# HaoZhongkai/DPOT

Hardware: AMD Instinct MI355X
Metric: PDE samples/sec (128^2 x10 -> 1 rollout step), DPOT-Tiny train step (higher is better)
Workload: dtype f32

## Files before the change

dpot_amd/_lib.py:

```python
from __future__ import annotations

import ctypes as C
import os
import threading

HERE = os.path.dirname(os.path.abspath(__file__))
LIB_PATH = os.environ.get("DPOT_HIP_LIB") or os.path.join(HERE, "lib", "libdpot_hip.so")

c_fp = C.c_void_p
c_i = C.c_int
c_i64 = C.c_int64
c_f = C.c_float
c_d = C.c_double


class GemmDesc(C.Structure):
    _fields_ = [
        ("A", c_fp), ("B", c_fp), ("C", c_fp),
        ("M", C.c_int32), ("N", C.c_int32), ("K", C.c_int32),
        ("batch", C.c_int32),
        ("transA", C.c_int32), ("transB", C.c_int32),
        ("lda", C.c_int32), ("ldb", C.c_int32), ("ldc", C.c_int32),
        ("strideA", c_i64), ("strideB", c_i64), ("strideC", c_i64),
        ("bias", c_fp), ("strideBias", c_i64),
# ... 76 lines not shown
    "dpot_groupnorm_ws_elems": (c_i64, [c_i] * 4),
    "dpot_groupnorm_fwd": (c_i, [c_fp] * 7 + [c_i] * 4 + [c_f, c_fp]),
    "dpot_groupnorm_bwd": (c_i, [c_fp] * 11 + [c_i] * 4 + [c_fp]),
    "dpot_groupnorm_bwd_packs_supported": (c_i, [c_i] * 3),
    "dpot_groupnorm_bwd_packs_rows": (c_i, [c_i] * 4),
    "dpot_groupnorm_bwd_packs": (c_i, [c_fp] * 12 + [c_i] * 4 + [c_fp]),
    "dpot_groupnorm_param_grads": (c_i, [C.c_void_p] * 3 + [c_i] * 3 + [c_fp]),
    "dpot_afno_fused_supported": (c_i, [c_i] * 7),
    "dpot_afno_fused_fwd": (c_i, [c_fp] * 19 + [c_i] * 9 + [c_f, c_fp]),
    "dpot_gn_dft_supported": (c_i, [c_i] * 4),
    "dpot_gn_rfft2": (c_i, [c_fp] * 6 + [c_i] * 8 + [c_f, c_fp]),
    "dpot_irfft2_gn": (c_i, [c_fp] * 12 + [c_i] * 9 + [c_f, c_fp]),
    "dpot_gn_bwd_rfft2": (c_i, [c_fp] * 8 + [c_i] * 9 + [c_fp]),
    "dpot_irfft2_gn_bwd": (c_i, [c_fp] * 9 + [c_i] * 9 + [c_fp]),
    "dpot_patchify": (c_i, [c_fp] * 5 + [c_i] * 6 + [c_fp]),
    "dpot_unpatchify": (c_i, [c_fp] * 2 + [c_i] * 6 + [c_fp]),
    "dpot_pixel_shuffle": (c_i, [c_fp] * 2 + [c_i] * 6 + [c_fp]),
    "dpot_copy2d_pad": (c_i, [c_fp, c_i, c_i, c_fp, c_i, c_i, c_fp]),
    "dpot_transpose2d": (c_i, [c_fp, c_fp, c_i, c_i, c_i, c_fp]),
    "dpot_colsum_parts": (c_i, [c_i]),
    "dpot_colsum": (c_i, [c_fp, c_i, c_i, c_i, c_fp, c_fp, c_fp]),
    "dpot_colsum_scatter": (c_i, [c_fp, c_i, c_i, c_i, c_fp, c_i, C.POINTER(C.c_int), C.POINTER(C.c_int),
                                  C.POINTER(C.c_void_p), c_fp]),
    "dpot_group_rowsum": (c_i, [c_fp, c_fp] + [c_i] * 4 + [c_fp]),
    "dpot_small_linear_supported": (c_i, [c_i] * 3),
    "dpot_small_linear": (c_i, [c_fp, c_i, c_fp, c_i, c_fp, c_fp, c_fp] + [c_i] * 5 + [c_fp]),
    "dpot_token_mean": (c_i, [c_fp, c_fp] + [c_i] * 3 + [c_fp]),
    "dpot_token_mean_bwd": (c_i, [c_fp] * 3 + [c_i] * 3 + [c_fp]),
    "dpot_bias_add": (c_i, [c_fp] * 3 + [c_i, c_i, c_fp]),
    "dpot_scale_shift": (c_i, [c_fp] * 4 + [c_i] * 3 + [c_fp]),
    "dpot_scale_shift_bwd": (c_i, [c_fp] * 6 + [c_i] * 3 + [c_fp]),
    "dpot_timeagg_scale_w": (c_i, [c_fp] * 4 + [c_i, c_i, c_fp]),
    "dpot_timeagg_scale_w_bwd": (c_i, [c_fp] * 6 + [c_i, c_i, c_fp]),
    "dpot_out_tail_partial_rows": (c_i, [c_i] * 4),
    "dpot_out_tail_partial_cols": (c_i, []),
    "dpot_out_tail_fwd": (c_i, [c_fp] * 6 + [c_i] * 6 + [c_fp]),
    "dpot_out_tail_bwd": (c_i, [c_fp] * 7 + [c_i] * 6 + [c_fp]),
    "dpot_rel_l2_chunks": (c_i, [c_i, c_i]),
    "dpot_rel_l2_fwd": (c_i, [c_fp] * 5 + [c_i] * 4 + [c_fp]),
    "dpot_rel_l2_bwd": (c_i, [c_fp] * 6 + [c_i] * 4 + [c_fp]),
    "dpot_sumsq": (c_i, [c_fp, c_i64, c_fp, c_fp, c_i, c_fp]),
    "dpot_adam_step": (c_i, [c_fp] * 4 + [c_i64, c_fp, c_fp, c_f, c_fp]),
    "dpot_adam_stage": (c_i, [c_fp, c_fp, c_f, c_d, c_d, c_f, c_f, c_f, c_i, c_fp]),
    "dpot_lamb_chunk_elems": (c_i, []),
    "dpot_lamb_step": (c_i, [c_fp] * 5 + [c_fp, c_f, c_fp, c_i, c_fp, c_i, c_fp, c_fp, c_i, c_fp]),
    "dpot_lamb_stage": (c_i, [c_fp, c_fp, c_d, c_d, c_d, c_f, c_f, c_f, c_f, c_i, c_i, c_fp]),
    "dpot_cls_ce_fwd": (c_i, [c_fp] * 4 + [c_i, c_i, c_fp]),
    "dpot_cls_ce_bwd": (c_i, [c_fp] * 5 + [c_i, c_i, c_fp]),
    "dpot_rel_l2_combine": (c_i, [c_fp, c_fp, c_i64, c_i, c_i, c_i, c_fp, c_fp]),
    "dpot_metrics_accum": (c_i, [c_fp] * 4 + [c_i, c_fp, c_f, c_i64, c_i64, c_i64, c_fp]),
    "dpot_noise_chunks": (c_i, [c_i, c_i]),
    "dpot_noise_inject": (c_i, [c_fp] * 4 + [c_f] + [c_i] * 3 + [c_fp]),
    "dpot_noise_inject_rng": (c_i, [c_fp] * 4 + [c_f] + [c_i] * 3 + [c_fp]),
    "dpot_noise_inject_bwd": (c_i, [c_fp] * 7 + [c_f] + [c_i] * 3 + [c_fp]),
    "dpot_window_slide": (c_i, [c_fp] * 3 + [c_i64] + [c_i] * 3 + [c_fp]),
    "dpot_window_slide_bwd": (c_i, [c_fp] * 3 + [c_i64] + [c_i] * 3 + [c_fp]),
    "dpot_resize_pad_window": (c_i, [c_fp, c_i, c_fp, c_fp] + [c_i] * 6 + [c_fp]),
    "dpot_spectral_resize_pad": (c_i, [c_i, c_i]),
    "dpot_spectral_resize": (c_i, [c_fp] * 7 + [c_i] * 6 + [c_fp]),
    "dpot_eval_metrics_pad": (c_i, [c_i, c_i]),
    "dpot_eval_metrics_max_size": (c_i, [c_i]),
    "dpot_eval_metrics_acc_elems": (c_i64, [c_i] * 4),
    "dpot_eval_metrics_stats": (c_i, [c_fp] * 9 + [c_i] * 4 + [c_fp]),
    "dpot_eval_metrics_finalize": (c_i, [c_fp] * 3 + [c_i] * 5 + [c_fp]),
    "dpot_panel_pack_weights": (c_i, [c_fp, c_i, c_i, c_fp]),
    "dpot_layout_jobs": (c_i, [c_fp, c_i, c_i64, c_fp]),
# ... 71 lines not shown
```

dpot_amd/build.py:

```python
from __future__ import annotations

import os
import shutil
import subprocess
import sys
from concurrent.futures import ThreadPoolExecutor

HERE = os.path.dirname(os.path.abspath(__file__))
CSRC = os.path.join(HERE, "csrc")
LIBDIR = os.path.join(HERE, "lib")
LIB = os.path.join(LIBDIR, "libdpot_hip.so")
SOURCES = ["core.hip", "gemm.hip", "gemm_panel.hip", "gemm_tn.hip", "gemm_bf16p.hip", "afno_mlp.hip", "afno_mlp6.hip", "afno_fused.hip", "dft.hip", "norm.hip", "gn_dft.hip", "misc.hip", "loss_opt.hip", "metrics.hip", "tail.hip", "data.hip", "embed.hip", "resize.hip", "evalmetrics.hip"]
FLAGS = ["--offload-arch=gfx950", "-O3", "-std=c++17", "-fPIC", "-Wall", "-Wno-unused-function",
         "-Wno-pass-failed"]
EXTRA_FLAGS = {"afno_mlp6.hip": ["-fno-slp-vectorize"]}


def _hipcc() -> str:
    for cand in (os.environ.get("HIPCC"), shutil.which("hipcc"), "/opt/rocm/bin/hipcc"):
        if cand and os.path.exists(cand):
            return cand
    raise RuntimeError("hipcc not found (need ROCm >= 7.0 to build the gfx950 kernels)")


def _stale(target: str, deps) -> bool:
    if not os.path.exists(target):
        return True
    t = os.path.getmtime(target)
    return any(os.path.getmtime(d) > t for d in deps)


def build(force: bool = False, verbose: bool = True) -> str:
    hipcc = _hipcc()
    os.makedirs(LIBDIR, exist_ok=True)
    hdrs = [os.path.join(CSRC, "common.h"), os.path.join(CSRC, "dft_fast.h"), os.path.join(CSRC, "gemm_split.h"), os.path.join(CSRC, "gemm_epi.h"), os.path.join(CSRC, "gemm_bf16p_common.h"), os.path.join(os.path.dirname(HERE), "include", "dpot_hip.h")]
    objs, jobs = [], []
    for src in SOURCES:
        s = os.path.join(CSRC, src)
        o = os.path.join(LIBDIR, src.replace(".hip", ".o"))
        objs.append(o)
        if force or _stale(o, [s] + hdrs):
            jobs.append([hipcc] + FLAGS + EXTRA_FLAGS.get(src, []) + ["-c", s, "-o", o])

    def run(cmd):
        if verbose:
# ... 17 lines not shown
```

dpot_amd/functional.py:

```python
from __future__ import annotations

import os
from collections import OrderedDict
from typing import Optional

import torch

from . import ops
from .ops import EPI_ACT, EPI_DACT

Tensor = torch.Tensor


def _pad4(n: int) -> int:
    return (n + 3) // 4 * 4


class _Sink:
    __slots__ = ("fp", "i")

    def __init__(self, param: Optional[Tensor], needed: bool):
        s = getattr(param, "_dpot_grad_slot", None) if (needed and param is not None) else None
        self.fp, self.i = s if s is not None else (None, -1)
        if self.fp is not None:
# ... 44 lines not shown
    return [_Sink(p, ctx.needs_input_grad[first_index + k]) for k, p in enumerate(params)]


def embed_grid_matrix(gx, gy, gt, X: int, Y: int, T: int, Cc: int, P: int):
    z = torch.zeros(1, X, Y, T, Cc, dtype=torch.float32, device=gx.device)
    return ops.patchify(z, gx, gy, gt, P)[:, Cc * P * P:].contiguous()


def embed_layout_jobs(pos, w0, b0, w2, b2):
    hid, E = w0.shape[0], w2.shape[0]
    K0 = w0[0].numel()
    hidp = _pad4(hid)
    tok = pos.shape[2] * pos.shape[3]
    return [(w0, None, (1, hidp, K0), (1, hid, K0), (0, K0, 1)),
            (b0, None, (1, 1, hidp), (1, 1, hid), (0, 0, 1)),
            (w2, None, (1, E, hidp), (1, E, hid), (0, hid, 1)),
            (pos, b2, (1, tok, E), (1, tok, E), (0, 1, tok))]


def embed_derived(pos, w0, b0, w2, b2, taw, tagamma, tt, T: int, grid=None, layouts=None):
    hid, E = w0.shape[0], w2.shape[0]
    K0 = w0[0].numel()
    hidp = _pad4(hid)
    tok = pos.shape[2] * pos.shape[3]
    dev = pos.device
    if layouts is not None:
        w0p, b0p, w2p, posb = layouts[0].view(hidp, K0), layouts[1].view(hidp), layouts[2].view(E, hidp), layouts[3].view(tok, E)
    else:
        w0p = ops.copy2d_pad(w0, hid, K0, hidp, K0)
        b0p = ops.copy2d_pad(b0, 1, hid, 1, hidp).view(hidp)
        w2p = ops.copy2d_pad(w2, E, hid, E, hidp)
        posT = ops.transpose2d(pos, 1, E, tok).view(tok, E)
        posb = ops.bias_add(posT, b2)
    ws = ops.timeagg_scale_w(taw, tagamma, tt) if tagamma is not None else taw
    V = torch.empty(T * hidp, E, dtype=torch.float32, device=dev)
    ops.gemm(w2p, ws, V, hidp, E, E, transA=True, lda=hidp, ldb=E, ldc=E, batch=T, strideA=0, strideB=E * E,
             strideC=hidp * E)
    wsum = ops.colsum(ws, T, E * E).view(E, E)
    cc = torch.empty(tok, E, dtype=torch.float32, device=dev)
    ops.gemm(posb, wsum, cc, tok, E, E, lda=E, ldb=E, ldc=E)
    wfrag = bt = None
    if grid is not None:
        kg = grid.shape[1]
        wfrag = ops.embed_pack_w0(w0)
        bt = torch.empty(grid.shape[0], hidp, dtype=torch.float32, device=dev)
        ops.gemm(grid, w0p[:, K0 - kg:], bt, grid.shape[0], hidp, kg, transB=True, lda=kg, ldb=K0, ldc=hidp, bias=b0p)
    return w0p, b0p, w2p, posb, ws, V, wsum, cc, wfrag, bt, grid


class EmbedFn(torch.autograd.Function):

    @staticmethod
    def forward(ctx, x, pos, w0, b0, w2, b2, taw, tagamma, gx, gy, gt, tt, P: int, act: int, derived=None):
        ops.capture_precision(ctx)
        x = x.contiguous()
        B, X, Y, T, Cc = x.shape
        h, w = X // P, Y // P
        tok = h * w
        hid, E = w0.shape[0], w2.shape[0]
        K0 = (Cc + 3) * P * P
        hidp = _pad4(hid)
        dev = x.device
        M = B * tok

        implicit = derived is not None and derived[8] is not None
        A0 = None if implicit else ops.patchify(x, gx, gy, gt, P)
        if derived is None:
            derived = embed_derived(pos, w0, b0, w2, b2, taw, tagamma, tt, T)
        w0p, b0p, w2p, posb, ws, V, wsum, cc, wfrag, bt, grid = derived
        if implicit:
            Hh, Hpre = ops.embed_fwd(x, wfrag, bt, hidp, act)
        else:
            Hh, Hpre = ops.linear_fwd(A0, w0p, b0p, act=act, save_pre=True)
        Yl = torch.empty(M, E, dtype=torch.float32, device=dev)
        ops.gemm(Hh, V, Yl, M, E, T * hidp, lda=T * hidp, ldb=E, ldc=E, res=cc, ldres=E, res_mod=tok)
        ctx.implicit = implicit
        ctx.save_for_backward(x if implicit else A0, Hpre, Hh, w0p, w2p, ws, V, wsum, posb, taw, tagamma, tt,
                              grid if implicit else x.new_empty(0))
        ctx.dims = (B, X, Y, T, Cc, P, h, w, hid, hidp, E, K0, act)
        ctx.sinks = _sinks(ctx, (pos, w0, b0, w2, b2, taw, tagamma), 1)
        ctx.weights_epoch = _epoch_of(ctx.sinks)
        return Yl.view(B, tok, E)

    @staticmethod
    @ops.with_ctx_precision
    def backward(ctx, dY):
        _check_epoch(ctx, "EmbedFn")
        A0, Hpre, Hh, w0p, w2p, ws, V, wsum, posb, taw, tagamma, tt, grid = ctx.saved_tensors
        B, X, Y, T, Cc, P, h, w, hid, hidp, E, K0, act = ctx.dims
        s_pos, s_w0, s_b0, s_w2, s_b2, s_taw, s_gamma = ctx.sinks
        tok = h * w
        M, M0 = B * tok, B * tok * T
        dev = dY.device
        dY = dY.contiguous().view(M, E)
        dHpre = torch.empty(M0, hidp, dtype=torch.float32, device=dev)
        ops.gemm(dY, V, dHpre, M, T * hidp, E, transB=True, lda=E, ldb=E, ldc=T * hidp, act=act, mode=EPI_DACT,
                 aux=Hpre, ldaux=T * hidp)
        dV = torch.empty(T * hidp, E, dtype=torch.float32, device=dev)
        ops.gemm(Hh, dY, dV, T * hidp, E, M, transA=True, lda=T * hidp, ldb=E, ldc=E,
                 splitk=ops.auto_splitk(T * hidp, E, M, tn=True))
        dc = ops.group_rowsum(dY, B, tok, 1, E)
        dwsum = torch.empty(E, E, dtype=torch.float32, device=dev)
        ops.gemm(posb, dc, dwsum, E, E, tok, transA=True, lda=E, ldb=E, ldc=E, splitk=ops.auto_splitk(E, E, tok, tn=True))
        dposb = torch.empty(tok, E, dtype=torch.float32, device=dev)
        ops.gemm(dc, wsum, dposb, tok, E, E, transB=True, lda=E, ldb=E, ldc=E)
        dpos = s_pos.done(ops.transpose2d(dposb, 1, tok, E, out=s_pos.out()).view(1, E, h, w))
        db2 = s_b2.done(ops.colsum(dposb, tok, E, out=s_b2.out()))
        dw2_t = torch.empty(T, E, hidp, dtype=torch.float32, device=dev)
        ops.gemm(ws, dV, dw2_t, E, hidp, E, transB=True, lda=E, ldb=E, ldc=hidp, batch=T, strideA=E * E,
                 strideB=hidp * E, strideC=E * hidp)
        dw2p = ops.colsum(dw2_t, T, E * hidp).view(E, hidp)
        dw2 = s_w2.done(ops.copy2d_pad(dw2p, E, hidp, E, hid, out=s_w2.out()).view(E, hid, 1, 1))
        dws = s_taw.out() if tagamma is None else None
        dws = ops._out(dws, (T, E, E), dev)
        ops.gemm(w2p, dV, dws, E, E, hidp, lda=hidp, ldb=E, ldc=E, batch=T, strideA=0, strideB=hidp * E,
                 strideC=E * E, res=dwsum, ldres=E, strideRes=0)
        if tagamma is not None:
            dtaw, dgamma = ops.timeagg_scale_w_bwd(dws, taw, tagamma, tt, out_dw=s_taw.out(),
                                                   out_dgamma=s_gamma.out())
            dtaw, dgamma = s_taw.done(dtaw), s_gamma.done(dgamma)
        else:
            dtaw, dgamma = s_taw.done(dws), None
        if ctx.implicit:
            db0 = s_b0.done(ops.colsum(dHpre, M0, hid, ld=hidp, out=s_b0.out()))
            dw0 = ops._out(s_w0.out(), (hid, K0), dev)
            ops.embed_wgrad(A0, dHpre, dw0, hid)
            dHs = ops.group_rowsum(dHpre, B, tok * T, 1, hidp)
            kg = grid.shape[1]
            ops.gemm(dHs, grid, dw0[:, K0 - kg:], hid, kg, tok * T, transA=True, lda=hidp, ldb=kg, ldc=K0)
            dw0 = s_w0.done(dw0.view(hid, Cc + 3, P, P))
        elif hid == hidp:
            dw0p, db0 = ops.linear_bwd_wb(dHpre, A0, None, s_b0.out())
            db0 = s_b0.done(db0)
        else:
            db0 = s_b0.done(ops.colsum(dHpre, M0, hid, ld=hidp, out=s_b0.out()))
            dw0p = ops.linear_bwd_weight(dHpre, A0)
        if not ctx.implicit:
            dw0 = s_w0.done(ops.copy2d_pad(dw0p, hidp, K0, hid, K0, out=s_w0.out()).view(hid, Cc + 3, P, P))
        dx = None
        if ctx.needs_input_grad[0]:
            dA0 = ops.linear_bwd_data(dHpre, w0p)
            dx = ops.unpatchify(dA0, B, X, Y, T, Cc, P)
        return dx, dpos, dw0, db0, dw2, db2, dtaw, dgamma, None, None, None, None, None, None, None


X6_MIN_FLOP = 3.0e9


def mlp_pack_kind(E: int, mh: int, M: Optional[int] = None) -> Optional[str]:
    eff = ops.effective_mlp_precision()
    Mq = 128 if M is None else M
    bf_ok = ops.gemm_bf16p_supported(Mq, mh, E) and ops.gemm_bf16p_supported(Mq, E, mh)
    if bf_ok and eff == ops.GEMM_BF16:
        return "bf16"
    if eff == ops.GEMM_F32 and ops.panel_enabled() and ops.gemm_panel_supported(Mq, mh, E) \
            and ops.gemm_panel_supported(Mq, E, mh):
        return "f32"
    return None


# ... 635 lines not shown
```

dpot_amd/ops.py:

```python
from __future__ import annotations

import ctypes as C
import contextlib
import functools
import threading
import os
from typing import Optional, Tuple

import torch

from . import _lib
from ._lib import GemmDesc, check

Tensor = torch.Tensor

ACT_IDS = {None: 0, "none": 0, "gelu": 1, "tanh": 2, "sigmoid": 3, "relu": 4, "leaky_relu": 5, "softplus": 6,
           "ELU": 7, "silu": 8}
EPI_LINEAR, EPI_ACT, EPI_DACT, EPI_AFNO_WGRAD = 0, 1, 2, 3
GEMM_F32, GEMM_BF16X6, GEMM_AUTO, GEMM_BF16 = 0, 1, 2, 3
_PRECISIONS = {"f32": GEMM_F32, "bf16x6": GEMM_BF16X6, "auto": GEMM_AUTO, "bf16": GEMM_BF16}
_gemm_precision = _PRECISIONS[os.environ.get("DPOT_GEMM_PRECISION", "f32")]


def set_gemm_precision(name: str) -> None:
# ... 72 lines not shown
        with precision_scope(getattr(ctx, "gemm_precision", None), getattr(ctx, "mlp_precision", None)):
            return backward(ctx, *grads)
    return wrapper


def capture_precision(ctx) -> None:
    ctx.gemm_precision = _cur_gemm()
    ctx.mlp_precision = effective_mlp_precision()


def effective_mlp_precision() -> int:
    m = _cur_mlp()
    return m if m is not None else _cur_gemm()


def mlp_precision() -> Optional[int]:
    return _cur_mlp()


TUNE_KEYS = {
    "mixer": (3, "AFNO mixer MLP: 3 = three-product fused kernel (afno_mlp3), 4 = four-product fused kernel (afno_mlp2), "
                 "0 = two generic GEMM launches"),
    "afno_layer": (-1, "one-launch AFNO layer forward (afno_fused_fwd): -1 = where it measured faster (>= 80 % full last "
                       "round of (sample, block) workgroups), 0 = never, 1 = wherever supported"),
    "gn_fuse": (1, "0 = GroupNorm as its own kernels: not fused with the mixer's DFTs, never applied on the load of its consumer"),
    "panel": (1, "0 = generic GEMM kernels instead of the pre-packed-weight panel GEMM, the token-contraction weight-gradient "
                 "kernels (gemm_tn) and their two-layer launches"),
    "wgrad_gauss": (1, "0 = four-product AFNO weight gradients instead of the three-product forms"),
    "bf16p_bd": (1, "0 = the LDS-DMA bf16 GEMM kernels of rounds 2-3 for every launch instead of the B-direct kernels"),
    "bf16p_shape": (1, "0 = none of the bf16 GEMM shape heuristics: 128 x 256 tiles only, column-major tile order, eight waves, "
                       "un-paired weight gradients"),
    "packs": (1, "0 = bf16 packs by separate pack passes only: none from the one-launch AFNO layer, the GroupNorm backward or Adam"),
    "pack_both": (1, "0 = bf16 channel MLP without the pack-both path (one pack pass per operand form, fp32 pre-activation saved)"),
    "fused_small": (1, "0 = separate small launches: per-block reduce launches, eight layout launches, torch ops for the cls head"),
    "embed_implicit": (1, "0 = explicit patch matrix + GEMM instead of the implicit-GEMM patch embedding"),
    "mixer6": (1, "bf16x6 mixer kernel afno_mlp6 under gemm_precision 'auto' / 'bf16x6': 1 = where it measured faster (96 channels "
                  "per block: DPOT-L), 2 = wherever supported (also 128), 0 = never (the fp32 matrix-core kernels)"),
}


_tune_parsed = ("", {})


def _parse_tune():
    global _tune_parsed
    env = os.environ.get("DPOT_TUNE", "")
    if env == _tune_parsed[0]:
        return _tune_parsed[1]
    out = {}
    for kv in env.split(","):
        kv = kv.strip()
        if not kv:
            continue
        k, _, v = kv.partition("=")
        if k not in TUNE_KEYS:
            raise ValueError(f"DPOT_TUNE: unknown key {k!r} (known: {', '.join(TUNE_KEYS)})")
        out[k] = int(v)
    _tune_parsed = (env, out)
    return out


def tune(key: str, default: Optional[int] = None) -> int:
    d = TUNE_KEYS[key][0] if default is None else default
    return _parse_tune().get(key, d)


def _stream() -> int:
# ... 837 lines not shown


def tile_vec(v: Tensor, reps: int) -> Tensor:
    N = v.numel()
    y = torch.empty(reps * N, dtype=torch.float32, device=v.device)
    check(_lib.load().dpot_bias_add(None, v.data_ptr(), y.data_ptr(), reps, N, _stream()), "tile_vec")
    return y


def scale_shift(x: Tensor, scale: Tensor, shift: Tensor) -> Tensor:
    B, T, E = x.shape
    y = torch.empty_like(x)
    check(_lib.load().dpot_scale_shift(x.data_ptr(), scale.data_ptr(), shift.data_ptr(), y.data_ptr(), B, T, E,
                                       _stream()), "scale_shift")
    return y


def scale_shift_bwd(dy: Tensor, x: Tensor, scale: Tensor):
    B, T, E = x.shape
    dx = torch.empty_like(x)
    dscale = torch.empty(B, E, dtype=torch.float32, device=x.device)
    dshift = torch.empty_like(dscale)
    check(_lib.load().dpot_scale_shift_bwd(dy.data_ptr(), x.data_ptr(), scale.data_ptr(), dx.data_ptr(),
                                           dscale.data_ptr(), dshift.data_ptr(), B, T, E, _stream()), "scale_shift_bwd")
    return dx, dscale, dshift


def timeagg_scale_w(w: Tensor, gamma: Tensor, tt: Tensor) -> Tensor:
    T, E, _ = w.shape
    ws = torch.empty_like(w)
    check(_lib.load().dpot_timeagg_scale_w(w.data_ptr(), gamma.data_ptr(), tt.data_ptr(), ws.data_ptr(), T, E,
                                           _stream()), "timeagg_scale_w")
    return ws


def timeagg_scale_w_bwd(dws: Tensor, w: Tensor, gamma: Tensor, tt: Tensor, out_dw: Optional[Tensor] = None,
                        out_dgamma: Optional[Tensor] = None) -> Tuple[Tensor, Tensor]:
    T, E, _ = w.shape
    dw = _out(out_dw, (T, E, E), w.device)
    dgamma = _out(out_dgamma, (1, E), w.device)
    check(_lib.load().dpot_timeagg_scale_w_bwd(dws.data_ptr(), w.data_ptr(), gamma.data_ptr(), tt.data_ptr(),
                                               dw.data_ptr(), dgamma.data_ptr(), T, E, _stream()),
          "timeagg_scale_w_bwd")
    return dw, dgamma


def out_tail_supported(old: int, co: int, n_pixels: int) -> bool:
    return old == 32 and 0 < co <= 32 and n_pixels % 32 == 0


def out_tail_pad(w4: Tensor, b4: Tensor, co: int) -> Tuple[Tensor, Tensor]:
    return copy2d_pad(w4, co, 32, 32, 32), copy2d_pad(b4, 1, co, 1, 32).view(32)


def out_tail_fwd(upre: Tensor, w2: Tensor, b2: Tensor, w4p: Tensor, b4p: Tensor, B: int, h: int, w: int, P: int,
                 co: int, act: int) -> Tensor:
    out = torch.empty(B, h * P, w * P, co, dtype=torch.float32, device=upre.device)
    check(_lib.load().dpot_out_tail_fwd(upre.data_ptr(), w2.data_ptr(), b2.data_ptr(), w4p.data_ptr(),
                                        b4p.data_ptr(), out.data_ptr(), B, h, w, P, co, act, _stream()), "out_tail_fwd")
    return out


def colsum_scatter(X: Tensor, M: int, N: int, segments) -> None:
    lib = _lib.load()
    n = len(segments)
    starts = (C.c_int * n)(*[s for s, _ in segments])
# ... 612 lines not shown
```

include/dpot_hip.h:

```cpp
#ifndef DPOT_HIP_H
#define DPOT_HIP_H

#include <stdint.h>

#ifdef __cplusplus
extern "C" {
#endif

#define DPOT_OK 0
#define DPOT_EINVAL (-1)
#define DPOT_EUNSUP (-2)
#define DPOT_EHIP (-3)

typedef void* dpot_stream_t;

enum {
  DPOT_ACT_NONE = 0,
  DPOT_ACT_GELU = 1,
  DPOT_ACT_TANH = 2,
  DPOT_ACT_SIGMOID = 3,
  DPOT_ACT_RELU = 4,
  DPOT_ACT_LEAKY_RELU = 5,
  DPOT_ACT_SOFTPLUS = 6,
  DPOT_ACT_ELU = 7,
// ... 137 lines not shown
int dpot_embed_supported(int C, int P, int T, int hid, int w);
int dpot_embed_wfrag_elems(void);
int dpot_embed_pack_w0(const float* w0, int hid, float* wfrag, dpot_stream_t stream);
int dpot_embed_fwd(const float* x, const float* wfrag, const float* btab, float* hpre, float* hh, int B, int X, int Y,
                   int T, int hidp, int act, dpot_stream_t stream);
int dpot_embed_wgrad_ws_elems(int B, int X, int Y);
int dpot_embed_wgrad(const float* x, const float* dhpre, float* workspace, float* dw0, int ldw, int hid, int B, int X,
                     int Y, int T, int hidp, dpot_stream_t stream);
int dpot_pixel_shuffle(const float* z, float* out, int B, int h, int w, int P, int Cc, int inverse,
                       dpot_stream_t stream);
int dpot_copy2d_pad(const float* src, int sR, int sC, float* dst, int dR, int dC, dpot_stream_t stream);
int dpot_transpose2d(const float* src, float* dst, int nbatch, int R, int C, dpot_stream_t stream);
int dpot_colsum_parts(int M);
int dpot_colsum(const float* X, int M, int N, int ld, float* out, float* part, dpot_stream_t stream);
int dpot_colsum_scatter(const float* X, int M, int N, int ld, float* part, int nseg, const int* seg_start,
                        const int* seg_len, float* const* seg_dst, dpot_stream_t stream);
int dpot_group_rowsum(const float* X, float* out, int B, int R, int T, int N, dpot_stream_t stream);
int dpot_token_mean(const float* x, float* y, int B, int T, int E, dpot_stream_t stream);
int dpot_token_mean_bwd(const float* dy, const float* add, float* dx, int B, int T, int E,
                        dpot_stream_t stream);
int dpot_small_linear_supported(int M, int N, int K);
int dpot_small_linear(const float* x, int ldx, const float* W, int ldw, const float* bias, float* y, float* pre, int ldy,
                      int M, int N, int K, int act, dpot_stream_t stream);
int dpot_bias_add(const float* x, const float* v, float* y, int R, int N, dpot_stream_t stream);
int dpot_scale_shift(const float* x, const float* scale, const float* shift, float* y, int B, int T, int E,
                     dpot_stream_t stream);
int dpot_scale_shift_bwd(const float* dy, const float* x, const float* scale, float* dx, float* dscale,
                         float* dshift, int B, int T, int E, dpot_stream_t stream);

int dpot_timeagg_scale_w(const float* w, const float* gamma, const float* tt, float* ws, int T, int E,
                         dpot_stream_t stream);
int dpot_timeagg_scale_w_bwd(const float* dws, const float* w, const float* gamma, const float* tt, float* dw,
                             float* dgamma, int T, int E, dpot_stream_t stream);

int dpot_out_tail_partial_rows(int B, int h, int w, int P);
int dpot_out_tail_partial_cols(void);
int dpot_out_tail_fwd(const float* upre, const float* w2, const float* b2, const float* w4, const float* b4,
                      float* out, int B, int h, int w, int P, int co, int act, dpot_stream_t stream);
int dpot_out_tail_bwd(const float* upre, const float* dout, const float* w2, const float* b2, const float* w4,
                      float* dupre, float* partials, int B, int h, int w, int P, int co, int act,
                      dpot_stream_t stream);

int dpot_rel_l2_chunks(int S, int C);
int dpot_rel_l2_fwd(const float* x, const float* y, const float* mask, float* stats, float* loss, int B,
                    int S, int C, int Tt, dpot_stream_t stream);
int dpot_rel_l2_bwd(const float* x, const float* y, const float* mask, const float* stats,
                    const float* gloss, float* dx, int B, int S, int C, int Tt, dpot_stream_t stream);

int dpot_sumsq(const float* g, int64_t n, float* out, float* part, int accumulate, dpot_stream_t stream);
int dpot_adam_step(float* p, const float* g, float* m, float* v, int64_t n, const float* hyper,
                   const float* sumsq, float grad_scale, dpot_stream_t stream);

int dpot_adam_stage(float* hyper, int64_t* step, float lr, double beta1, double beta2, float eps,
                    float weight_decay, float max_norm, int advance, dpot_stream_t stream);

typedef struct dpot_lamb_chunk {
  int64_t off;
  int32_t len, tensor;
} dpot_lamb_chunk;
typedef struct dpot_lamb_tensor {
  int32_t first_chunk, n_chunks;
} dpot_lamb_tensor;
int dpot_lamb_chunk_elems(void);
int dpot_lamb_step(float* p, const float* g, float* m, float* v, const float* hyper, const float* sumsq, float grad_scale,
                   const dpot_lamb_chunk* chunks_dev, int nchunks, const dpot_lamb_tensor* tensors_dev, int ntensors,
                   double* part, float* norms, int adam, dpot_stream_t stream);
// ... 134 lines not shown
```

Measured before the change: 10610.

## Fuse embed-stage time-aggregation scaling, reductions and weight-grad GEMM into merged kernels

Adds embed_fold kernels that merge several small launches in the embedding stage. The forward pass computes the cosine-scaled time-aggregation weights and their sum over time in one pass, replacing the separate timeagg_scale_w and colsum launches. The backward pass runs the dc row-sum, the dHs row-sum and the db0 column-sum in one launch. A matrix-core kernel computes dws together with dtaw and the dgamma partials, so dws is never written to memory, and a final kernel reduces dgamma and db0. This cuts launch count and memory traffic in a small stage, but adds more custom code and the risk that the MFMA kernel is less efficient than the tuned GEMM.

New measurement: 10480. 1.2% lower.

```diff
diff --git a/dpot_amd/_lib.py b/dpot_amd/_lib.py
--- a/dpot_amd/_lib.py
+++ b/dpot_amd/_lib.py
@@ -132,6 +132,12 @@
     "dpot_scale_shift_bwd": (c_i, [c_fp] * 6 + [c_i] * 3 + [c_fp]),
     "dpot_timeagg_scale_w": (c_i, [c_fp] * 4 + [c_i, c_i, c_fp]),
     "dpot_timeagg_scale_w_bwd": (c_i, [c_fp] * 6 + [c_i, c_i, c_fp]),
+    "dpot_embed_fold_supported": (c_i, [c_i] * 5),
+    "dpot_embed_fold_fwd_a": (c_i, [c_fp] * 5 + [c_i, c_i, c_fp]),
+    "dpot_embed_fold_db0_parts": (c_i, [c_i, c_i]),
+    "dpot_embed_fold_bwd_a": (c_i, [c_fp] * 5 + [c_i] * 6 + [c_fp]),
+    "dpot_embed_fold_bwd_c": (c_i, [c_fp] * 8 + [c_i] * 3 + [c_fp]),
+    "dpot_embed_fold_bwd_fin": (c_i, [c_fp, c_fp, c_i, c_fp, c_i, c_i, c_fp, c_fp]),
     "dpot_out_tail_partial_rows": (c_i, [c_i] * 4),
     "dpot_out_tail_partial_cols": (c_i, []),
     "dpot_out_tail_fwd": (c_i, [c_fp] * 6 + [c_i] * 6 + [c_fp]),
diff --git a/dpot_amd/build.py b/dpot_amd/build.py
--- a/dpot_amd/build.py
+++ b/dpot_amd/build.py
@@ -10,7 +10,7 @@
 CSRC = os.path.join(HERE, "csrc")
 LIBDIR = os.path.join(HERE, "lib")
 LIB = os.path.join(LIBDIR, "libdpot_hip.so")
-SOURCES = ["core.hip", "gemm.hip", "gemm_panel.hip", "gemm_tn.hip", "gemm_bf16p.hip", "afno_mlp.hip", "afno_mlp6.hip", "afno_fused.hip", "dft.hip", "norm.hip", "gn_dft.hip", "misc.hip", "loss_opt.hip", "metrics.hip", "tail.hip", "data.hip", "embed.hip", "resize.hip", "evalmetrics.hip"]
+SOURCES = ["core.hip", "gemm.hip", "gemm_panel.hip", "gemm_tn.hip", "gemm_bf16p.hip", "afno_mlp.hip", "afno_mlp6.hip", "afno_fused.hip", "dft.hip", "norm.hip", "gn_dft.hip", "misc.hip", "loss_opt.hip", "metrics.hip", "tail.hip", "data.hip", "embed.hip", "embed_fold.hip", "resize.hip", "evalmetrics.hip"]
 FLAGS = ["--offload-arch=gfx950", "-O3", "-std=c++17", "-fPIC", "-Wall", "-Wno-unused-function",
          "-Wno-pass-failed"]
 EXTRA_FLAGS = {"afno_mlp6.hip": ["-fno-slp-vectorize"]}
diff --git a/dpot_amd/csrc/embed_fold.hip b/dpot_amd/csrc/embed_fold.hip
--- /dev/null
+++ b/dpot_amd/csrc/embed_fold.hip
@@ -0,0 +1,297 @@
+#include "common.h"
+
+namespace dpot {
+
+typedef float fold_f32x16 __attribute__((ext_vector_type(16)));
+
+constexpr int FOLD_TMAX = 12;
+
+template <int CW>
+__device__ __forceinline__ void fold_colsum_block(const float* __restrict__ X, int M, int N, int ld, float* __restrict__ out,
+                                                  int rows_per_part, int bx, int by, float* red ) {
+  constexpr int RL = 256 / CW;
+  const int tc = threadIdx.x % CW, tr = threadIdx.x / CW;
+  const int n = bx * CW + tc;
+  const int m0 = by * rows_per_part;
+  int m1 = m0 + rows_per_part;
+  if (m1 > M) m1 = M;
+  float s0 = 0.f, s1 = 0.f, s2 = 0.f, s3 = 0.f;
+  if (n < N) {
+    const float* p = X + n;
+    int m = m0 + tr;
+    for (; m + 3 * RL < m1; m += 4 * RL) {
+      s0 += p[(long long)m * ld];
+      s1 += p[(long long)(m + RL) * ld];
+      s2 += p[(long long)(m + 2 * RL) * ld];
+      s3 += p[(long long)(m + 3 * RL) * ld];
+    }
+    for (; m < m1; m += RL) s0 += p[(long long)m * ld];
+  }
+  red[tr * CW + tc] = (s0 + s1) + (s2 + s3);
+  __syncthreads();
+  if (tr == 0 && n < N) {
+    float s = 0.f;
+#pragma unroll
+    for (int r = 0; r < RL; ++r) s += red[r * CW + tc];
+    out[(long long)by * N + n] = s;
+  }
+}
+__device__ __forceinline__ void fold_colsum_any(int cw, const float* X, int M, int N, int ld, float* out, int rpp, int bx,
+                                                int by, float* red) {
+  if (cw == 16) fold_colsum_block<16>(X, M, N, ld, out, rpp, bx, by, red);
+  else if (cw == 32) fold_colsum_block<32>(X, M, N, ld, out, rpp, bx, by, red);
+  else fold_colsum_block<64>(X, M, N, ld, out, rpp, bx, by, red);
+}
+static int fold_colsum_cw(int N) { return N <= 16 ? 16 : N <= 32 ? 32 : 64; }
+
+__device__ __forceinline__ void fold_rowsum_block(const float* __restrict__ X, float* __restrict__ out, int B, int R, int N,
+                                                  int bx, int by, float* red ) {
+  const int tc = threadIdx.x & 63, tr = threadIdx.x >> 6;
+  const int n = bx * 64 + tc;
+  const int r = by;
+  float s0 = 0.f, s1 = 0.f;
+  if (n < N) {
+    int q = tr;
+    for (; q + 4 < B; q += 8) {
+      s0 += X[((long long)q * R + r) * N + n];
+      s1 += X[((long long)(q + 4) * R + r) * N + n];
+    }
+    for (; q < B; q += 4) s0 += X[((long long)q * R + r) * N + n];
+  }
+  red[tr * 64 + tc] = s0 + s1;
+  __syncthreads();
+  if (tr == 0 && n < N) out[(long long)r * N + n] = (red[tc] + red[64 + tc]) + (red[128 + tc] + red[192 + tc]);
+}
+
+__global__ __launch_bounds__(256) void embed_fold_fwd_a_kernel(const float* __restrict__ w, const float* __restrict__ gamma,
+                                                               const float* __restrict__ tt, float* __restrict__ ws,
+                                                               float* __restrict__ wsum, int T, int E) {
+  __shared__ float cs[FOLD_TMAX];
+  const int i = blockIdx.x;
+  if (threadIdx.x < T) cs[threadIdx.x] = cosf(tt[threadIdx.x] * gamma[i]);
+  __syncthreads();
+  int full[4];
+#pragma unroll
+  for (int k = 0; k < 4; ++k) full[k] = (T > k ? (T - k + 3) / 4 : 0) & ~3;
+  for (int j = threadIdx.x; j < E; j += 256) {
+    float s[4][4];
+#pragma unroll
+    for (int k = 0; k < 4; ++k)
+#pragma unroll
+      for (int u = 0; u < 4; ++u) s[k][u] = 0.f;
+#pragma unroll
+    for (int t = 0; t < FOLD_TMAX; ++t) {
+      if (t < T) {
+        const long long off = ((long long)t * E + i) * E + j;
+        const float x = w[off] * cs[t];
+        ws[off] = x;
+        const int k = t & 3, p = t >> 2;
+        if (p < full[k]) s[k][p & 3] += x;
+        else s[k][0] += x;
+      }
+    }
+    float r = 0.f;
+#pragma unroll
+    for (int k = 0; k < 4; ++k) r += (s[k][0] + s[k][1]) + (s[k][2] + s[k][3]);
+    wsum[(long long)i * E + j] = r;
+  }
+}
+
+struct FoldBwdA {
+  const float* dY;
+  const float* dHpre;
+  float* dc;
+  float* dHs;
+  float* db0_out;
+  int B, tok, T, E, hid, hidp;
+  int parts, rpp, cw;
+  int n_dc, n_dhs;
+};
+__global__ __launch_bounds__(256) void embed_fold_bwd_a_kernel(const FoldBwdA p) {
+  __shared__ float red[256];
+  int bid = blockIdx.x;
+  if (bid < p.n_dc) {
+    const int nx = p.E / 64;
+    fold_rowsum_block(p.dY, p.dc, p.B, p.tok, p.E, bid % nx, bid / nx, red);
+    return;
+  }
+  bid -= p.n_dc;
+  if (bid < p.n_dhs) {
+    const int nx = (p.hidp + 63) / 64;
+    fold_rowsum_block(p.dHpre, p.dHs, p.B, p.tok * p.T, p.hidp, bid % nx, bid / nx, red);
+    return;
+  }
+  bid -= p.n_dhs;
+  const int nx = (p.hid + p.cw - 1) / p.cw;
+  fold_colsum_any(p.cw, p.dHpre, p.B * p.tok * p.T, p.hid, p.hidp, p.db0_out, p.rpp, bid % nx, bid / nx, red);
+}
+
+struct FoldBwdC {
+  const float* w2p;
+  const float* dV;
+  const float* dwsum;
+  const float* taw;
+  const float* gamma;
+  const float* tt;
+  float* dtaw;
+  float* P;
+  int T, E, hidp, cgroups;
+};
+__global__ __launch_bounds__(256) void embed_fold_bwd_c_kernel(const FoldBwdC p) {
+  __shared__ float cs_tab[FOLD_TMAX][32], coef_tab[FOLD_TMAX][32];
+  __shared__ float s_tab[FOLD_TMAX][16][64];
+  const int tid = threadIdx.x, lane = tid & 63, wave = tid >> 6;
+  const int li = lane & 31, kh = lane >> 5;
+  const int i0 = (blockIdx.x / p.cgroups) * 32, c0 = (blockIdx.x % p.cgroups) * 32;
+  const int E = p.E, hidp = p.hidp;
+  const bool has_gamma = p.gamma != nullptr;
+  if (has_gamma) {
+    for (int idx = tid; idx < p.T * 32; idx += 256) {
+      const int t = idx >> 5, r = idx & 31;
+      const float tv = p.tt[t];
+      const float arg = tv * p.gamma[i0 + r];
+      cs_tab[t][r] = cosf(arg);
+      coef_tab[t][r] = -sinf(arg) * tv;
+    }
+  }
+  __syncthreads();
+  for (int t = wave; t < p.T; t += 4) {
+    float s[16];
+#pragma unroll
+    for (int r = 0; r < 16; ++r) s[r] = 0.f;
+    for (int j0 = c0; j0 < E; j0 += 256) {
+      fold_f32x16 acc;
+#pragma unroll
+      for (int r = 0; r < 16; ++r) acc[r] = 0.f;
+      const float* arow = p.w2p + (long long)(i0 + li) * hidp;
+      const float* bcol = p.dV + (long long)t * hidp * E + j0 + li;
+      for (int kk = 0; kk < hidp; kk += 8) {
+        const int k = kk + 4 * kh;
+        float4 a = make_float4(0.f, 0.f, 0.f, 0.f), b = a;
+        if (k < hidp) {
+          a = *reinterpret_cast<const float4*>(arow + k);
+          b.x = bcol[(long long)(k + 0) * E];
+          b.y = bcol[(long long)(k + 1) * E];
+          b.z = bcol[(long long)(k + 2) * E];
+          b.w = bcol[(long long)(k + 3) * E];
+        }
+        acc = __builtin_amdgcn_mfma_f32_32x32x2f32(a.x, b.x, acc, 0, 0, 0);
+        acc = __builtin_amdgcn_mfma_f32_32x32x2f32(a.y, b.y, acc, 0, 0, 0);
+        acc = __builtin_amdgcn_mfma_f32_32x32x2f32(a.z, b.z, acc, 0, 0, 0);
+        acc = __builtin_amdgcn_mfma_f32_32x32x2f32(a.w, b.w, acc, 0, 0, 0);
+      }
+      const int j = j0 + li;
+#pragma unroll
+      for (int r = 0; r < 16; ++r) {
+        const int row = (r & 3) + 8 * (r >> 2) + 4 * kh;
+        const long long ij = (long long)(i0 + row) * E + j;
+        const float d = acc[r] + p.dwsum[ij];
+        const long long off = (long long)t * E * E + ij;
+        if (has_gamma) {
+          p.dtaw[off] = d * cs_tab[t][row];
+          s[r] = fmaf(d, p.taw[off], s[r]);
+        } else {
+          p.dtaw[off] = d;
+        }
+      }
+    }
+    if (has_gamma) {
+#pragma unroll
+      for (int r = 0; r < 16; ++r) s_tab[t][r][lane] = s[r];
+    }
+  }
+  __syncthreads();
+  if (has_gamma && wave == 0) {
+#pragma unroll
+    for (int r = 0; r < 16; ++r) {
+      const int row = (r & 3) + 8 * (r >> 2) + 4 * kh;
+      float acc = 0.f;
+      for (int t = 0; t < p.T; ++t) acc = fmaf(s_tab[t][r][lane], coef_tab[t][row], acc);
+      p.P[(long long)(i0 + row) * 256 + c0 + li] = acc;
+    }
+  }
+}
+
+__global__ __launch_bounds__(256) void embed_fold_bwd_fin_kernel(const float* __restrict__ P, float* __restrict__ dgamma,
+                                                                 int n_gamma, int pvalid, const float* __restrict__ part,
+                                                                 int parts, int hid, int cw, float* __restrict__ db0) {
+  __shared__ float red[256];
+  int bid = blockIdx.x;
+  if (bid < n_gamma) {
+    const float v = (int)threadIdx.x < pvalid ? P[(long long)bid * 256 + threadIdx.x] : 0.f;
+    const float dg = block_sum(v, red);
+    if (threadIdx.x == 0) dgamma[bid] = dg;
+    return;
+  }
+  bid -= n_gamma;
+  fold_colsum_any(cw, part, parts, hid, hid, db0, parts, bid, 0, red);
+}
+
+}
+
+using namespace dpot;
+
+extern "C" int dpot_embed_fold_supported(int T, int E, int hid, int hidp, int tok) {
+  return T >= 1 && T <= FOLD_TMAX && E >= 64 && E % 64 == 0 && hid >= 1 && hidp >= hid && hidp % 4 == 0 && hidp <= 128 &&
+         tok >= 16 && tok % 16 == 0 && tok <= 65535;
+}
+
+extern "C" int dpot_embed_fold_fwd_a(const float* taw, const float* gamma, const float* tt, float* ws, float* wsum, int T,
+                                     int E, dpot_stream_t stream) {
+  DPOT_REQUIRE(taw && gamma && tt && ws && wsum, "embed_fold_fwd_a: bad argument");
+  if (!(T >= 1 && T <= FOLD_TMAX && E >= 64 && E % 64 == 0)) return DPOT_EUNSUP;
+  hipLaunchKernelGGL(embed_fold_fwd_a_kernel, dim3(E), dim3(256), 0, as_stream(stream), taw, gamma, tt, ws, wsum, T, E);
+  return check_launch("embed_fold_fwd_a_kernel");
+}
+
+extern "C" int dpot_embed_fold_db0_parts(int M0, int hid) {
+  int parts = dpot_colsum_parts(M0);
+  const int want = cdiv(1024, cdiv(hid, fold_colsum_cw(hid)));
+  if (parts > want) parts = want;
+  return parts < 1 ? 1 : parts;
+}
+
+extern "C" int dpot_embed_fold_bwd_a(const float* dY, const float* dHpre, float* dc, float* dHs, float* db0_out, int B,
+                                     int tok, int T, int E, int hid, int hidp, dpot_stream_t stream) {
+  DPOT_REQUIRE(dY && dc && B > 0 && (!dHpre || (dHs && db0_out)), "embed_fold_bwd_a: bad argument");
+  if (!dpot_embed_fold_supported(T, E, hid, hidp, tok)) return DPOT_EUNSUP;
+  const long long M0 = (long long)B * tok * T;
+  if (M0 > 0x7fffffffll / hidp) return DPOT_EUNSUP;
+  FoldBwdA p;
+  p.dY = dY; p.dHpre = dHpre; p.dc = dc; p.dHs = dHs; p.db0_out = db0_out;
+  p.B = B; p.tok = tok; p.T = T; p.E = E; p.hid = hid; p.hidp = hidp;
+  p.cw = fold_colsum_cw(hid);
+  p.parts = dpot_embed_fold_db0_parts((int)M0, hid);
+  p.rpp = cdiv((int)M0, p.parts);
+  p.n_dc = (E / 64) * tok;
+  p.n_dhs = dHpre ? cdiv(hidp, 64) * tok * T : 0;
+  const int n_db0 = dHpre ? cdiv(hid, p.cw) * p.parts : 0;
+  hipLaunchKernelGGL(embed_fold_bwd_a_kernel, dim3(p.n_dc + p.n_dhs + n_db0), dim3(256), 0, as_stream(stream), p);
+  return check_launch("embed_fold_bwd_a_kernel");
+}
+
+extern "C" int dpot_embed_fold_bwd_c(const float* w2p, const float* dV, const float* dwsum, const float* taw,
+                                     const float* gamma, const float* tt, float* dtaw, float* P, int T, int E, int hidp,
+                                     dpot_stream_t stream) {
+  DPOT_REQUIRE(w2p && dV && dwsum && dtaw && (!gamma || (taw && tt && P)), "embed_fold_bwd_c: bad argument");
+  if (!(T >= 1 && T <= FOLD_TMAX && E >= 64 && E % 64 == 0 && hidp >= 4 && hidp % 4 == 0 && hidp <= 128 &&
+        aligned16(w2p)))
+    return DPOT_EUNSUP;
+  FoldBwdC p;
+  p.w2p = w2p; p.dV = dV; p.dwsum = dwsum; p.taw = taw; p.gamma = gamma; p.tt = tt; p.dtaw = dtaw; p.P = P;
+  p.T = T; p.E = E; p.hidp = hidp;
+  p.cgroups = (E < 256 ? E : 256) / 32;
+  hipLaunchKernelGGL(embed_fold_bwd_c_kernel, dim3((E / 32) * p.cgroups), dim3(256), 0, as_stream(stream), p);
+  return check_launch("embed_fold_bwd_c_kernel");
+}
+
+extern "C" int dpot_embed_fold_bwd_fin(const float* P, float* dgamma, int E, const float* db0_part, int parts, int hid,
+                                       float* db0, dpot_stream_t stream) {
+  const int n_gamma = dgamma ? E : 0;
+  const int n_db0 = db0 ? cdiv(hid, fold_colsum_cw(hid)) : 0;
+  DPOT_REQUIRE((!dgamma || (P && E >= 64)) && (!db0 || (db0_part && parts >= 1 && hid >= 1)) && n_gamma + n_db0 > 0,
+               "embed_fold_bwd_fin: bad argument");
+  hipLaunchKernelGGL(embed_fold_bwd_fin_kernel, dim3(n_gamma + n_db0), dim3(256), 0, as_stream(stream), P, dgamma,
+                     n_gamma, E < 256 ? E : 256, db0_part, parts, hid > 0 ? hid : 1, fold_colsum_cw(hid > 0 ? hid : 1), db0);
+  return check_launch("embed_fold_bwd_fin_kernel");
+}
diff --git a/dpot_amd/functional.py b/dpot_amd/functional.py
--- a/dpot_amd/functional.py
+++ b/dpot_amd/functional.py
@@ -100,11 +100,16 @@
         w2p = ops.copy2d_pad(w2, E, hid, E, hidp)
         posT = ops.transpose2d(pos, 1, E, tok).view(tok, E)
         posb = ops.bias_add(posT, b2)
-    ws = ops.timeagg_scale_w(taw, tagamma, tt) if tagamma is not None else taw
+    fold = tagamma is not None and ops.embed_fold_enabled(T, E, hid, hidp, tok)
+    if fold:
+        ws, wsum = ops.embed_fold_fwd_a(taw, tagamma, tt)
+    else:
+        ws = ops.timeagg_scale_w(taw, tagamma, tt) if tagamma is not None else taw
     V = torch.empty(T * hidp, E, dtype=torch.float32, device=dev)
     ops.gemm(w2p, ws, V, hidp, E, E, transA=True, lda=hidp, ldb=E, ldc=E, batch=T, strideA=0, strideB=E * E,
              strideC=hidp * E)
-    wsum = ops.colsum(ws, T, E * E).view(E, E)
+    if not fold:
+        wsum = ops.colsum(ws, T, E * E).view(E, E)
     cc = torch.empty(tok, E, dtype=torch.float32, device=dev)
     ops.gemm(posb, wsum, cc, tok, E, E, lda=E, ldb=E, ldc=E)
     wfrag = bt = None
@@ -167,7 +172,13 @@
         dV = torch.empty(T * hidp, E, dtype=torch.float32, device=dev)
         ops.gemm(Hh, dY, dV, T * hidp, E, M, transA=True, lda=T * hidp, ldb=E, ldc=E,
                  splitk=ops.auto_splitk(T * hidp, E, M, tn=True))
-        dc = ops.group_rowsum(dY, B, tok, 1, E)
+        fold = ops.embed_fold_enabled(T, E, hid, hidp, tok)
+        dHs = db0_job = None
+        if fold:
+            dc, dHs, db0_job = ops.embed_fold_bwd_a(dY, dHpre if ctx.implicit else None, B, tok, T, E, hid, hidp,
+                                                    out_db0=s_b0.out() if ctx.implicit else None)
+        else:
+            dc = ops.group_rowsum(dY, B, tok, 1, E)
         dwsum = torch.empty(E, E, dtype=torch.float32, device=dev)
         ops.gemm(posb, dc, dwsum, E, E, tok, transA=True, lda=E, ldb=E, ldc=E, splitk=ops.auto_splitk(E, E, tok, tn=True))
         dposb = torch.empty(tok, E, dtype=torch.float32, device=dev)
@@ -179,21 +190,32 @@
                  strideB=hidp * E, strideC=E * hidp)
         dw2p = ops.colsum(dw2_t, T, E * hidp).view(E, hidp)
         dw2 = s_w2.done(ops.copy2d_pad(dw2p, E, hidp, E, hid, out=s_w2.out()).view(E, hid, 1, 1))
-        dws = s_taw.out() if tagamma is None else None
-        dws = ops._out(dws, (T, E, E), dev)
-        ops.gemm(w2p, dV, dws, E, E, hidp, lda=hidp, ldb=E, ldc=E, batch=T, strideA=0, strideB=hidp * E,
-                 strideC=E * E, res=dwsum, ldres=E, strideRes=0)
-        if tagamma is not None:
-            dtaw, dgamma = ops.timeagg_scale_w_bwd(dws, taw, tagamma, tt, out_dw=s_taw.out(),
-                                                   out_dgamma=s_gamma.out())
-            dtaw, dgamma = s_taw.done(dtaw), s_gamma.done(dgamma)
-        else:
-            dtaw, dgamma = s_taw.done(dws), None
+        if fold:
+            dtaw, Pg = ops.embed_fold_bwd_c(w2p, dV, dwsum, taw, tagamma, tt, out_dw=s_taw.out())
+            dgamma = ops.embed_fold_bwd_fin(Pg, E, db0_job if ctx.implicit else None,
+                                            out_dgamma=s_gamma.out() if tagamma is not None else None)
+            dtaw = s_taw.done(dtaw)
+            dgamma = s_gamma.done(dgamma) if tagamma is not None else None
+        else:
+            dws = s_taw.out() if tagamma is None else None
+            dws = ops._out(dws, (T, E, E), dev)
+            ops.gemm(w2p, dV, dws, E, E, hidp, lda=hidp, ldb=E, ldc=E, batch=T, strideA=0, strideB=hidp * E,
+                     strideC=E * E, res=dwsum, ldres=E, strideRes=0)
+            if tagamma is not None:
+                dtaw, dgamma = ops.timeagg_scale_w_bwd(dws, taw, tagamma, tt, out_dw=s_taw.out(),
+                                                       out_dgamma=s_gamma.out())
+                dtaw, dgamma = s_taw.done(dtaw), s_gamma.done(dgamma)
+            else:
+                dtaw, dgamma = s_taw.done(dws), None
         if ctx.implicit:
-            db0 = s_b0.done(ops.colsum(dHpre, M0, hid, ld=hidp, out=s_b0.out()))
+            if fold:
+                db0 = s_b0.done(db0_job[0])
+            else:
+                db0 = s_b0.done(ops.colsum(dHpre, M0, hid, ld=hidp, out=s_b0.out()))
             dw0 = ops._out(s_w0.out(), (hid, K0), dev)
             ops.embed_wgrad(A0, dHpre, dw0, hid)
-            dHs = ops.group_rowsum(dHpre, B, tok * T, 1, hidp)
+            if not fold:
+                dHs = ops.group_rowsum(dHpre, B, tok * T, 1, hidp)
             kg = grid.shape[1]
             ops.gemm(dHs, grid, dw0[:, K0 - kg:], hid, kg, tok * T, transA=True, lda=hidp, ldb=kg, ldc=K0)
             dw0 = s_w0.done(dw0.view(hid, Cc + 3, P, P))
diff --git a/dpot_amd/ops.py b/dpot_amd/ops.py
--- a/dpot_amd/ops.py
+++ b/dpot_amd/ops.py
@@ -128,7 +128,8 @@
                        "un-paired weight gradients"),
     "packs": (1, "0 = bf16 packs by separate pack passes only: none from the one-launch AFNO layer, the GroupNorm backward or Adam"),
     "pack_both": (1, "0 = bf16 channel MLP without the pack-both path (one pack pass per operand form, fp32 pre-activation saved)"),
-    "fused_small": (1, "0 = separate small launches: per-block reduce launches, eight layout launches, torch ops for the cls head"),
+    "fused_small": (1, "0 = separate small launches: per-block reduce launches, eight layout launches, torch ops for the cls head, "
+                       "the embed stage without the merged launches of csrc/embed_fold.hip"),
     "embed_implicit": (1, "0 = explicit patch matrix + GEMM instead of the implicit-GEMM patch embedding"),
     "mixer6": (1, "bf16x6 mixer kernel afno_mlp6 under gemm_precision 'auto' / 'bf16x6': 1 = where it measured faster (96 channels "
                   "per block: DPOT-L), 2 = wherever supported (also 128), 0 = never (the fp32 matrix-core kernels)"),
@@ -1032,6 +1033,61 @@
     check(_lib.load().dpot_timeagg_scale_w(w.data_ptr(), gamma.data_ptr(), tt.data_ptr(), ws.data_ptr(), T, E,
                                            _stream()), "timeagg_scale_w")
     return ws
+
+
+def embed_fold_enabled(T: int, E: int, hid: int, hidp: int, tok: int) -> bool:
+    return (tune("fused_small") != 0 and _cur_gemm() in (GEMM_F32, GEMM_AUTO)
+            and bool(_lib.load().dpot_embed_fold_supported(T, E, hid, hidp, tok)))
+
+
+def embed_fold_fwd_a(w: Tensor, gamma: Tensor, tt: Tensor) -> Tuple[Tensor, Tensor]:
+    T, E, _ = w.shape
+    ws = torch.empty_like(w)
+    wsum = torch.empty(E, E, dtype=torch.float32, device=w.device)
+    check(_lib.load().dpot_embed_fold_fwd_a(w.data_ptr(), gamma.data_ptr(), tt.data_ptr(), ws.data_ptr(), wsum.data_ptr(),
+                                            T, E, _stream()), "embed_fold_fwd_a")
+    return ws, wsum
+
+
+def embed_fold_bwd_a(dY: Tensor, dHpre: Optional[Tensor], B: int, tok: int, T: int, E: int, hid: int, hidp: int,
+                     out_db0: Optional[Tensor] = None):
+    lib = _lib.load()
+    dev = dY.device
+    dc = torch.empty(tok, E, dtype=torch.float32, device=dev)
+    dHs = db0 = part = None
+    parts = 1
+    if dHpre is not None:
+        dHs = torch.empty(tok * T, hidp, dtype=torch.float32, device=dev)
+        db0 = _out(out_db0, (hid,), dev)
+        parts = lib.dpot_embed_fold_db0_parts(B * tok * T, hid)
+        part = torch.empty(parts, hid, dtype=torch.float32, device=dev) if parts > 1 else None
+    check(lib.dpot_embed_fold_bwd_a(dY.data_ptr(), _p(dHpre), dc.data_ptr(), _p(dHs), _p(part if parts > 1 else db0),
+                                    B, tok, T, E, hid, hidp, _stream()), "embed_fold_bwd_a")
+    return dc, dHs, (db0, part, parts)
+
+
+def embed_fold_bwd_c(w2p: Tensor, dV: Tensor, dwsum: Tensor, w: Tensor, gamma: Optional[Tensor], tt: Tensor,
+                     out_dw: Optional[Tensor] = None) -> Tuple[Tensor, Optional[Tensor]]:
+    T, E, _ = w.shape
+    hidp = w2p.shape[1]
+    dw = _out(out_dw, (T, E, E), w.device)
+    P = torch.empty(E, 256, dtype=torch.float32, device=w.device) if gamma is not None else None
+    check(_lib.load().dpot_embed_fold_bwd_c(w2p.data_ptr(), dV.data_ptr(), dwsum.data_ptr(), w.data_ptr(), _p(gamma),
+                                            tt.data_ptr(), dw.data_ptr(), _p(P), T, E, hidp, _stream()), "embed_fold_bwd_c")
+    return dw, P
+
+
+def embed_fold_bwd_fin(P: Optional[Tensor], E: int, db0_job=None, out_dgamma: Optional[Tensor] = None) -> Optional[Tensor]:
+    db0, part, parts = db0_job if db0_job is not None else (None, None, 1)
+    dgamma = _out(out_dgamma, (1, E), P.device) if P is not None else None
+    if parts <= 1:
+        db0 = part = None
+    if dgamma is None and db0 is None:
+        return None
+    hid = db0.numel() if db0 is not None else 0
+    check(_lib.load().dpot_embed_fold_bwd_fin(_p(P), _p(dgamma), E, _p(part), parts, hid, _p(db0), _stream()),
+          "embed_fold_bwd_fin")
+    return dgamma
 
 
 def timeagg_scale_w_bwd(dws: Tensor, w: Tensor, gamma: Tensor, tt: Tensor, out_dw: Optional[Tensor] = None,
diff --git a/include/dpot_hip.h b/include/dpot_hip.h
--- a/include/dpot_hip.h
+++ b/include/dpot_hip.h
@@ -193,6 +193,17 @@
                          dpot_stream_t stream);
 int dpot_timeagg_scale_w_bwd(const float* dws, const float* w, const float* gamma, const float* tt, float* dw,
                              float* dgamma, int T, int E, dpot_stream_t stream);
+
+int dpot_embed_fold_supported(int T, int E, int hid, int hidp, int tok);
+int dpot_embed_fold_fwd_a(const float* taw, const float* gamma, const float* tt, float* ws, float* wsum, int T, int E,
+                          dpot_stream_t stream);
+int dpot_embed_fold_db0_parts(int M0, int hid);
+int dpot_embed_fold_bwd_a(const float* dY, const float* dHpre, float* dc, float* dHs, float* db0_out, int B, int tok,
+                          int T, int E, int hid, int hidp, dpot_stream_t stream);
+int dpot_embed_fold_bwd_c(const float* w2p, const float* dV, const float* dwsum, const float* taw, const float* gamma,
+                          const float* tt, float* dtaw, float* P, int T, int E, int hidp, dpot_stream_t stream);
+int dpot_embed_fold_bwd_fin(const float* P, float* dgamma, int E, const float* db0_part, int parts, int hid, float* db0,
+                            dpot_stream_t stream);
 
 int dpot_out_tail_partial_rows(int B, int h, int w, int P);
 int dpot_out_tail_partial_cols(void);
```
